# ZKTLabs/zkt-plonk

Hardware: AMD Instinct MI355X
Metric: proofs/sec (withdraw, n=2^20) (higher is better)
Workload: dtype u32 limbs (256-bit Montgomery); 1 GPU; full prove, WithdrawCircuit INPUTS=8 HEIGHT=64 Poseidon x5 (1019498 gates, 538 Poseidon gadgets), bn254, n=2^20, TABLE_SIZE=1024, 12 public inputs; parallelism=proofs sharded across 1 GPU(s), chained=True, distinct_witnesses=2, witness_on_device=True, table_cached=True, proof_bytes=802

## Files before the change

zkt-plonk_amd/csrc/kzg.hip:

```cpp
#include "ctx.hpp"
#include "hostinv.hpp"
#include "msm.hpp"
#include "poly.hpp"

#include <algorithm>
#include <cstring>
#include <functional>
#include <vector>

namespace zkt {

constexpr int KZG_OPEN_E = 4;

struct KzgState {
    hipStream_t copy = nullptr;
    hipEvent_t ev_up = nullptr, ev_main = nullptr;
    DevBuf up;
    DevBuf t, tb, w, scan, pw, part, evals;
    ~KzgState() {
        if (ev_up) (void)hipEventDestroy(ev_up);
        if (ev_main) (void)hipEventDestroy(ev_main);
        if (copy) (void)hipStreamDestroy(copy);
    }
};

static int kzg_state(zkt_ctx* c, KzgState** out) {
    if (!c->kzg) {
        auto K = std::make_shared<KzgState>();
        ZKT_HIP(c, hipStreamCreateWithFlags(&K->copy, hipStreamNonBlocking));
        ZKT_HIP(c, hipEventCreateWithFlags(&K->ev_up, hipEventDisableTiming));
        ZKT_HIP(c, hipEventCreateWithFlags(&K->ev_main, hipEventDisableTiming));
        c->kzg = K;
    }
// ... 100 lines not shown
};

template <class P>
ZKT_D Fe<P> wave_sum(Fe<P> x) {
#pragma unroll
    for (int d = 32; d >= 1; d >>= 1) {
        Fe<P> y;
#pragma unroll
        for (int w = 0; w < P::N; ++w) y.v[w] = (uint32_t)__shfl_xor((int)x.v[w], d, 64);
        x = fe_add<P>(x, y);
    }
    return x;
}

template <class P>
__global__ __launch_bounds__(256) void k_kzg_open_combine(KzgOpenArgs a, const Fe<P>* pw, const Fe<P>* blk, int fstride,
                                                         uint64_t len_max, int raw, Fe<P>* t_out, Fe<P>* partials, uint32_t nblk) {
    __shared__ Fe<P> wsum[ZKT_KZG_BATCH_MAX][4];
    const int t = threadIdx.x, lane = t & 63, wave = t >> 6;
    const uint64_t base = (uint64_t)blockIdx.x * 256 * KZG_OPEN_E;
    const Fe<P> z256 = fe_load<P>(pw + 256), zt = fe_load<P>(pw + t);
    Fe<P> acc[KZG_OPEN_E];
#pragma unroll
    for (int e = 0; e < KZG_OPEN_E; ++e) acc[e] = fe_zero<P>();
#pragma unroll 1
    for (int j = 0; j < a.nterms; ++j) {
        const uint64_t len = a.len[j];
        if (base >= len) {
            if (lane == 0) wsum[j][wave] = fe_zero<P>();
            continue;
        }
        const Fe<P>* p = (const Fe<P>*)a.poly[j];
        Fe<P> cj;
#pragma unroll
        for (int w = 0; w < P::N; ++w) cj.v[w] = a.ch[j][w];
        Fe<P> h = fe_zero<P>();
#pragma unroll
        for (int e = KZG_OPEN_E - 1; e >= 0; --e) {
            const uint64_t i = base + (uint64_t)e * 256 + t;
            const Fe<P> v = i < len ? fe_load<P>(p + i) : fe_zero<P>();
            h = fe_add<P>(fe_mul<P>(h, z256), v);
            acc[e] = fe_add<P>(acc[e], fe_mul<P>(cj, v));
        }
        h = wave_sum<P>(fe_mul<P>(h, zt));
        if (lane == 0) wsum[j][wave] = h;
    }
    const Fe<P> zb = fe_load<P>(blk + (size_t)fstride * blockIdx.x);
    Fe<P> r = fe_mul<P>(zb, zt);
#pragma unroll
    for (int e = 0; e < KZG_OPEN_E; ++e) {
        const uint64_t i = base + (uint64_t)e * 256 + t;
        if (i < len_max) fe_store<P>(t_out + i, raw ? acc[e] : fe_mul<P>(acc[e], r));
        r = fe_mul<P>(r, z256);
    }
    __syncthreads();
    if (t < a.nterms) {
        Fe<P> s = fe_add<P>(fe_add<P>(wsum[t][0], wsum[t][1]), fe_add<P>(wsum[t][2], wsum[t][3]));
        fe_store<P>(partials + (size_t)t * nblk + blockIdx.x, fe_mul<P>(s, zb));
    }
}

template <class P>
static int open_combine_t(zkt_ctx* c, const KzgOpenArgs& a, const void* pw, size_t len_max, int raw, void* t_out, void* partials,
                          uint32_t nblk) {
    const Fe<P>* tab = (const Fe<P>*)pw;
    const int fstride = KZG_OPEN_E / open_elems(len_max);
    hipLaunchKernelGGL(k_kzg_open_combine<P>, dim3(nblk), dim3(256), 0, c->stream, a, tab, tab + 2 * OPEN_PW_ROW, fstride, (uint64_t)len_max,
                       raw, (Fe<P>*)t_out, (Fe<P>*)partials, nblk);
    ZKT_HIP(c, hipGetLastError());
    return ZKT_OK;
}

template <class P>
static void inv_host(const uint32_t* z, uint32_t* zi) {
    Fe<P> x;
    memcpy(x.v, z, 32);
    x = fe_inv_host<P>(x);
    memcpy(zi, x.v, 32);
}

static int kzg_open(zkt_ctx* c, const void* const* src, bool host, const size_t* lens, int k, const uint64_t* ch, const uint64_t* z4,
                    uint64_t* out_w, int* out_inf, uint64_t* out_evals) {
    int rc = kzg_check(c, src, lens, k, out_w);
    if (rc || k == 0) return rc;
    if (!ch || !z4) return set_err(c, ZKT_ERR_INVALID_ARGUMENT, "null pointer");
    size_t L = 0, total = 0;
    for (int j = 0; j < k; ++j) {
        L = std::max(L, lens[j]);
        total += lens[j];
    }
    if (L > 0 && open_elems(L) > KZG_OPEN_E)
        return set_err(c, ZKT_ERR_INVALID_ARGUMENT, "zkt_kzg_open: polynomials longer than 2^26 coefficients");
    const int W = 2 * fq_limbs(c);
    std::vector<uint64_t> w(W, 0), ev((size_t)k * 4, 0);
    if (L == 0) {
        memcpy(out_w, w.data(), W * 8);
        if (out_inf) *out_inf = 1;
        if (out_evals) memcpy(out_evals, ev.data(), ev.size() * 8);
        return ZKT_OK;
    }
    (void)hipSetDevice(c->device);
    KzgState* K = nullptr;
    if ((rc = kzg_state(c, &K))) return rc;
    const uint32_t nblk = (uint32_t)((L + 256 * KZG_OPEN_E - 1) / (256 * KZG_OPEN_E));
    if ((rc = grow(c, K->t, L * 32)) || (rc = grow(c, K->tb, L * 32)) || (rc = grow(c, K->w, L * 32)) ||
        (rc = grow(c, K->scan, (2 * (L / 1024 + 2048)) * 32)) || (rc = grow(c, K->pw, open_witness_powers(L) * 32)) ||
        (rc = grow(c, K->part, (size_t)k * nblk * 32)) || (rc = grow(c, K->evals, (size_t)k * 32)))
        return rc;
    if (host && (rc = grow(c, K->up, total * 32))) return rc;
    KzgOpenArgs a{};
    a.nterms = k;
    size_t off = 0;
    for (int j = 0; j < k; ++j) {
        a.poly[j] = host ? (const void*)((char*)K->up.p + off) : src[j];
        a.len[j] = lens[j];
        memcpy(a.ch[j], ch + 4 * (size_t)j, 32);
        off += lens[j] * 32;
    }
    if (host) {
        if ((rc = kzg_copy_after_main(c, *K))) return rc;
        ProfScope prof(c, "kzg_open_upload", K->copy);
        for (int j = 0; j < k && !rc; ++j)
            if (lens[j]) rc = kzg_upload(c, *K, src[j], lens[j] * 32, const_cast<void*>(a.poly[j]));
        if (rc) return rc;
    }
    uint32_t z[8], zi[8] = {};
    memcpy(z, z4, 32);
    bool zero = true;
    for (int i = 0; i < 8; ++i) zero = zero && z[i] == 0;
    if (!zero) {
        if (c->curve == ZKT_CURVE_BN254) inv_host<Bn254Fr>(z, zi);
        else inv_host<Bls381Fr>(z, zi);
    }
    {
        ProfScope prof(c, "kzg_open_combine");
        if ((rc = open_pow_tables(c, z, zi, K->pw.p, L))) return rc;
        rc = c->curve == ZKT_CURVE_BN254 ? open_combine_t<Bn254Fr>(c, a, K->pw.p, L, zero, K->t.p, K->part.p, nblk)
                                         : open_combine_t<Bls381Fr>(c, a, K->pw.p, L, zero, K->t.p, K->part.p, nblk);
        if (rc) return rc;
        if (out_evals && (rc = poly_sum_rows(c, K->part.p, (int)nblk, k, K->evals.p))) return rc;
    }
    int inf = 1;
    if (L >= 2) {
        const void* scalars = (const char*)K->t.p + 32;
        if (!zero) {
            ProfScope prof(c, "kzg_open_divide");
            if ((rc = open_divide(c, K->t.p, L, K->tb.p, K->scan.p, K->w.p, K->pw.p))) return rc;
            scalars = K->w.p;
        }
        ProfScope prof(c, "kzg_open_msm");
        if ((rc = msm_g1_dev(c, scalars, L - 1, 0, 1, w.data(), &inf))) return rc;
    }
    if (out_evals) ZKT_HIP(c, hipMemcpyAsync(ev.data(), K->evals.p, (size_t)k * 32, hipMemcpyDeviceToHost, c->stream));
    ZKT_HIP(c, hipStreamSynchronize(c->stream));
    memcpy(out_w, w.data(), W * 8);
    if (out_inf) *out_inf = inf;
    if (out_evals) memcpy(out_evals, ev.data(), ev.size() * 8);
    return ZKT_OK;
}

}

// ... 24 lines not shown
```

zkt-plonk_amd/csrc/poly.hip:

```cpp
#include "poly.hpp"
#include "hostinv.hpp"

namespace zkt {

template <class P>
ZKT_D Fe<P> arg_fe(const uint32_t* w) {
    Fe<P> r;
#pragma unroll
    for (int i = 0; i < 8; ++i) r.v[i] = w[i];
    return r;
}

template <class P>
__global__ void k_mul_vec(const Fe<P>* a, const Fe<P>* b, Fe<P>* o, size_t n) {
    size_t i = (size_t)blockIdx.x * blockDim.x + threadIdx.x;
    if (i < n) fe_store<P>(o + i, fe_mul<P>(fe_load<P>(a + i), fe_load<P>(b + i)));
}

template <class P>
__global__ void k_trim_len(const Fe<P>* p, size_t lo, size_t n, uint32_t* len, int skip_if_set, Fe<P>* zero_at,
                           int zero_count) {
    if (zero_at && blockIdx.x == 0 && (int)threadIdx.x < zero_count) fe_store<P>(zero_at + threadIdx.x, fe_zero<P>());
    if (skip_if_set && *len != 0) return;
    size_t i = lo + (size_t)blockIdx.x * blockDim.x + threadIdx.x;
// ... 383 lines not shown

template <class P>
__global__ void k_quot_blind(Fe<P>* lo, Fe<P>* mid, Fe<P>* hi, const uint32_t* lens, const Fe<P>* b0b1, uint32_t n,
                             uint32_t* status) {
    if (threadIdx.x != 0 || blockIdx.x != 0) return;
    if (lens[3] > 3 * (n + 2)) { atomicOr(status, 2u); return; }
    if (lens[1] == 0 || lens[2] == 0) { atomicOr(status, 1u); return; }
    Fe<P> b0 = fe_load<P>(b0b1), b1 = fe_load<P>(b0b1 + 1);
    fe_store<P>(lo + lens[0], b0);
    fe_store<P>(mid, fe_sub<P>(fe_load<P>(mid), b0));
    fe_store<P>(mid + lens[1], b1);
    fe_store<P>(hi, fe_sub<P>(fe_load<P>(hi), b1));
}

constexpr int PW_E = 8;
constexpr int OW_THREADS = 1024;
static inline int ow_elems(size_t len) {
    int e = 2;
    while ((len + (size_t)256 * e - 1) / ((size_t)256 * e) > 65536) e <<= 1;
    return e;
}
static inline size_t ow_blocks(size_t len) {
    const size_t seg = (size_t)256 * ow_elems(len);
    return (len + seg - 1) / seg;
}
size_t open_witness_powers(size_t maxlen) { return 2 * (size_t)EV_PW + 2 * ow_blocks(maxlen) + 8; }

template <class P>
ZKT_D void pow_rounds(Fe<P>* tab, const Fe<P>& x, int cnt, int lt) {
    if (lt == 0) {
        tab[0] = fe_one<P>();
        tab[1] = x;
    }
    __syncthreads();
    for (int s = 1; s < cnt; s <<= 1) {
        for (int j = lt + 1; j <= s && s + j <= cnt; j += OW_THREADS / 2) tab[s + j] = fe_mul<P>(tab[s], tab[j]);
        __syncthreads();
    }
}
template <class P>
__global__ __launch_bounds__(OW_THREADS) void k_pow_tables(Fe<P> z, Fe<P> zinv, Fe<P>* pw, int nblk, int E) {
    __shared__ Fe<P> row[2][EV_PW], seg[2][EV_PW], top[2][EV_PW];
    const int half = threadIdx.x / (OW_THREADS / 2), lt = threadIdx.x % (OW_THREADS / 2);
    pow_rounds<P>(row[half], half ? zinv : z, 256, lt);
    Fe<P> y = row[half][256];
    for (int e = 1; e < E; e <<= 1) y = fe_sqr<P>(y);
    pow_rounds<P>(seg[half], y, 256, lt);
    const int ntop = (nblk + 255) / 256;
    pow_rounds<P>(top[half], seg[half][256], ntop, lt);
    for (int t = lt; t < EV_PW; t += OW_THREADS / 2) fe_store<P>(pw + half * EV_PW + t, row[half][t]);
    Fe<P>* blk = pw + 2 * EV_PW + (size_t)half * nblk;
    for (int b = lt; b < nblk; b += OW_THREADS / 2) fe_store<P>(blk + b, fe_mul<P>(seg[half][b & 255], top[half][b >> 8]));
}
template <class P>
__global__ __launch_bounds__(256) void k_mul_pow(const Fe<P>* in, Fe<P>* out, size_t n, size_t cap, const Fe<P>* pw, const Fe<P>* blk,
                                                 int E, int shift) {
    const size_t base = (size_t)blockIdx.x * 256 * E;
    Fe<P> r = fe_mul<P>(fe_load<P>(blk + blockIdx.x), fe_load<P>(pw + threadIdx.x + shift));
#pragma unroll 1
    for (int j = 0; j < E; ++j) {
        const size_t i = base + (size_t)j * 256 + threadIdx.x;
        if (i >= cap) break;
        fe_store<P>(out + i, i < n ? fe_mul<P>(fe_load<P>(in + i), r) : fe_zero<P>());
        if (j + 1 < E) r = fe_mul<P>(r, fe_load<P>(pw + 256));
    }
}

template <class P>
__global__ void k_gen_powers(Fe<P>* out, size_t n, Fe<P> base, Fe<P> scale) {
    size_t t = (size_t)blockIdx.x * blockDim.x + threadIdx.x;
    size_t i0 = t * PW_E;
    if (i0 >= n) return;
    Fe<P> pw = fe_mul<P>(scale, fe_pow_u64<P>(base, i0));
#pragma unroll 1
    for (int e = 0; e < PW_E && i0 + e < n; ++e) {
        fe_store<P>(out + i0 + e, pw);
        pw = fe_mul<P>(pw, base);
    }
}
// ... 389 lines not shown
    if ((rc = trim_len_t<P>(c, hi, chunk, lens + 2))) return rc;
    {
        const size_t lo = 3 * chunk, hi = 4 * n;
        hipLaunchKernelGGL(k_trim_len<P>, dim3(nblocks(hi - lo)), dim3(256), 0, c->stream, (const Fe<P>*)q, lo, hi, lens + 3, 0,
                           (Fe<P>*)nullptr, 0);
        ZKT_HIP(c, hipGetLastError());
    }
    hipLaunchKernelGGL(k_quot_blind<P>, dim3(1), dim3(64), 0, c->stream, (Fe<P>*)lo, (Fe<P>*)mid, (Fe<P>*)hi, lens, (const Fe<P>*)b0b1, (uint32_t)n, d_status);
    ZKT_HIP(c, hipGetLastError());
    return ZKT_OK;
}
int quotient_split_blind(zkt_ctx* c, const void* q, size_t n, const void* d_b0b1, void* q_lo, void* q_mid, void* q_hi, uint32_t* d_status) {
    ZKT_DISPATCH(c, quot_split_t, q, n, d_b0b1, q_lo, q_mid, q_hi, d_status);
}

int open_elems(size_t len) { return ow_elems(len); }
size_t open_blocks(size_t len) { return ow_blocks(len); }
template <class P> static int open_pow_tables_t(zkt_ctx* c, const uint32_t* z, const uint32_t* zinv, void* d_powers, size_t len) {
    hipLaunchKernelGGL(k_pow_tables<P>, dim3(1), dim3(OW_THREADS), 0, c->stream, host_fe<P>(z), host_fe<P>(zinv), (Fe<P>*)d_powers,
                       (int)ow_blocks(len), ow_elems(len));
    ZKT_HIP(c, hipGetLastError());
    return ZKT_OK;
}
int open_pow_tables(zkt_ctx* c, const uint32_t z[8], const uint32_t z_inv[8], void* d_powers, size_t len) {
    ZKT_DISPATCH(c, open_pow_tables_t, z, z_inv, d_powers, len);
}
template <class P> static int open_divide_t(zkt_ctx* c, const void* t, size_t len, void* tb, void* scan_tmp, void* out, const void* d_powers) {
    if (len == 0) return ZKT_OK;
    const Fe<P>* pw = (const Fe<P>*)d_powers;
    const int E = ow_elems(len);
    const unsigned blocks = (unsigned)ow_blocks(len);
    int rc = scan_t<P, OpAdd>(c, (const Fe<P>*)t, (Fe<P>*)tb, len, true, (Fe<P>*)scan_tmp);
    if (rc) return rc;
    hipLaunchKernelGGL(k_mul_pow<P>, dim3(blocks), dim3(256), 0, c->stream, (const Fe<P>*)tb + 1, (Fe<P>*)out, len - 1, len,
                       pw + EV_PW, pw + 2 * EV_PW + blocks, E, 1);
    ZKT_HIP(c, hipGetLastError());
    return ZKT_OK;
}
int open_divide(zkt_ctx* c, const void* t, size_t len, void* d_tmp, void* d_scan_tmp, void* out, const void* d_powers) {
    ZKT_DISPATCH(c, open_divide_t, t, len, d_tmp, d_scan_tmp, out, d_powers);
}

template <class P> static int open_witness_t(zkt_ctx* c, const void* p, size_t len, const uint32_t* z, const uint32_t* zinv, void* ta, void* tb, void* scan_tmp, void* out, void* d_powers) {
    if (len == 0) return ZKT_OK;
    Fe<P>* pw = (Fe<P>*)d_powers;
    const int E = ow_elems(len);
    const unsigned blocks = (unsigned)ow_blocks(len);
    int rc = open_pow_tables_t<P>(c, z, zinv, d_powers, len);
    if (rc) return rc;
    hipLaunchKernelGGL(k_mul_pow<P>, dim3(blocks), dim3(256), 0, c->stream, (const Fe<P>*)p, (Fe<P>*)ta, len, len,
                       (const Fe<P>*)pw, (const Fe<P>*)pw + 2 * EV_PW, E, 0);
    ZKT_HIP(c, hipGetLastError());
    return open_divide_t<P>(c, ta, len, tb, scan_tmp, out, d_powers);
}
int open_witness(zkt_ctx* c, const void* p, size_t len, const uint32_t z[8], const uint32_t z_inv[8], void* d_tmp_a, void* d_tmp_b, void* d_scan_tmp, void* out, void* d_powers) {
    ZKT_DISPATCH(c, open_witness_t, p, len, z, z_inv, d_tmp_a, d_tmp_b, d_scan_tmp, out, d_powers);
}

template <class P> static int sum_rows_t(zkt_ctx* c, const void* partials, int nblk, int rows, void* out) {
    hipLaunchKernelGGL(k_eval_final<P>, dim3(rows), dim3(256), 0, c->stream, (const Fe<P>*)partials, nblk, (Fe<P>*)out);
    ZKT_HIP(c, hipGetLastError());
    return ZKT_OK;
}
int poly_sum_rows(zkt_ctx* c, const void* d_partials, int nblk, int rows, void* d_out) {
    ZKT_DISPATCH(c, sum_rows_t, d_partials, nblk, rows, d_out);
}

template <class P> static int gen_powers_t(zkt_ctx* c, void* out, size_t n, const uint32_t* base, const uint32_t* scale) {
    if (!n) return ZKT_OK;
    hipLaunchKernelGGL(k_gen_powers<P>, dim3(nblocks((n + PW_E - 1) / PW_E)), dim3(256), 0, c->stream, (Fe<P>*)out, n, host_fe<P>(base), host_fe<P>(scale));
    ZKT_HIP(c, hipGetLastError());
// ... 32 lines not shown
```

zkt-plonk_amd/csrc/poly.hpp:

```cpp
#pragma once
#include "ctx.hpp"

namespace zkt {

constexpr int LC_MAX_TERMS = 16;
struct LinCombArgs {
    const void* poly[LC_MAX_TERMS];
    uint64_t len[LC_MAX_TERMS];
    uint32_t scalar[LC_MAX_TERMS][8];
    int nterms;
};

constexpr int EVAL_MAX = 16;
struct EvalArgs {
    const void* poly[EVAL_MAX];
    uint64_t len[EVAL_MAX];
    uint32_t point[EVAL_MAX][8];
    int count;
};

struct QuotientArgs {
    const void *a, *b, *c, *pi, *z1, *z2, *t, *h1, *h2;
    const void *q_m, *q_l, *q_r, *q_o, *q_c, *q_lookup, *q_table, *sigma1, *sigma2, *sigma3, *x, *l1;
    void* out;
// ... 25 lines not shown
int poly_add_blinders(zkt_ctx* c, void* p, const uint32_t* d_len, const void* d_blinders, int k, size_t cap);
int poly_lincomb(zkt_ctx* c, const LinCombArgs& a, void* out, size_t n);
int lagrange_scalars(zkt_ctx* c, const void* ev, size_t n, const uint32_t* d_len, const void* d_blinders, int k, const void* d_roots,
                     void* out);
int poly_eval_many(zkt_ctx* c, const EvalArgs& a, void* d_partials, void* d_results, void* d_powers);
int z1_terms(zkt_ctx* c, const ZTermsArgs& a);
int z2_terms(zkt_ctx* c, const ZTermsArgs& a);
int scan_mul(zkt_ctx* c, const void* in, void* out, size_t n, bool reverse, void* d_tmp );
int scan_add(zkt_ctx* c, const void* in, void* out, size_t n, bool reverse, void* d_tmp);
int z_combine(zkt_ctx* c, const void* pn, const void* sd, const uint32_t inv_total[8], void* out, size_t n);
int quotient_pointwise(zkt_ctx* c, const QuotientArgs& a);
int to_hat_form(zkt_ctx* c, void* v, size_t n, int k32);
int quotient_interleave(zkt_ctx* c, const void* in, void* out, size_t n4, uint32_t G, uint32_t chunks = 1);
int quotient_split_blind(zkt_ctx* c, const void* q, size_t n, const void* d_b0b1, void* q_lo, void* q_mid, void* q_hi,
                         uint32_t* d_status);
int open_witness(zkt_ctx* c, const void* p, size_t len, const uint32_t z[8], const uint32_t z_inv[8], void* d_tmp_a, void* d_tmp_b,
                 void* d_scan_tmp, void* out, void* d_powers );
size_t open_witness_powers(size_t maxlen);
constexpr int OPEN_PW_ROW = 257;
int open_elems(size_t len);
size_t open_blocks(size_t len);
int open_pow_tables(zkt_ctx* c, const uint32_t z[8], const uint32_t z_inv[8], void* d_powers, size_t len);
int open_divide(zkt_ctx* c, const void* t, size_t len, void* d_tmp, void* d_scan_tmp, void* out, const void* d_powers);
int poly_sum_rows(zkt_ctx* c, const void* d_partials, int nblk, int rows, void* d_out);
int gen_powers(zkt_ctx* c, void* out, size_t n, const uint32_t base[8], const uint32_t scale[8]);
int lookup_count(zkt_ctx* c, const void* f, size_t n, const void* d_sorted_keys, const uint32_t* d_perm, uint32_t nkeys,
                 uint32_t* d_counts, uint32_t* d_status);
int lookup_starts(zkt_ctx* c, const uint32_t* d_base_counts, uint32_t* d_hits, uint32_t nkeys, size_t n, uint32_t* d_even,
                  uint32_t* d_odd, uint32_t* d_status);
int lookup_expand(zkt_ctx* c, const void* d_keys_insertion, const uint32_t* d_starts, uint32_t nkeys, void* out, size_t n);

}
```

zkt-plonk_amd/csrc/prover.hip:

```cpp
#include "ctx.hpp"
#include "hostinv.hpp"
#include <chrono>
#include <cstdio>
#include <cstdlib>
#include "ec.hpp"
#include "keyfile.hpp"
#include "msm.hpp"
#include "poly.hpp"
#include "transcript.hpp"

#include <algorithm>
#include <functional>
#include <cstring>
#include <memory>
#include <optional>
#include <vector>

namespace zkt {

enum { PK_QM = 0, PK_QL, PK_QR, PK_QO, PK_QC, PK_S1, PK_S2, PK_S3, PK_QLOOKUP, PK_QTABLE, PK_COUNT };
enum { CS_QM = 0, CS_QL, CS_QR, CS_QO, CS_QC, CS_QLOOKUP, CS_QTABLE, CS_S1, CS_S2, CS_S3, CS_X, CS_L1, CS_COUNT };
enum { W_A = 0, W_B, W_C, W_PI, W_Z1, W_Z2, W_T, W_H1, W_H2, W_COUNT };

struct CircuitState {
// ... 26 lines not shown
    uint32_t lk_nkeys = 0;
    std::vector<uint32_t> lk_host_keys, lk_host_sorted, lk_host_counts, lk_host_order;
    bool has_next = false, prefetch_same_table = false;
    int prefetch_stage = 0;
    uint64_t prefetch_epoch = 0;
    zkt_prove_inputs next_in{}, prefetch_in{};
    void* poly_alt[3] = {};
    uint32_t* status_alt = nullptr;
    void* lk_keys = nullptr;
    size_t lk_cap = 0;
    void* pinned = nullptr;
    hipStream_t comm_stream = nullptr;
    hipEvent_t ev_piece[ZKT_QUOTIENT_CHUNKS] = {}, ev_gathered = nullptr;
    hipStream_t aux_stream = nullptr;
    hipEvent_t ev_aux_go = nullptr, ev_aux_done = nullptr;
    void* aux_scan_tmp = nullptr;
    void* aux_pw = nullptr;
    hipStream_t copy_stream = nullptr;
    hipEvent_t ev_copy[4] = {};
    void* pinned_pi = nullptr;
    uint32_t* pi_tab = nullptr;
    void* eval_pw = nullptr;
    std::vector<uint64_t> cached_table;
    bool t_cached = false, t_coset_valid = false;
    uint64_t t_srs_generation = 0;
    uint64_t t_commit_xy[12] = {};
    bool keys_borrowed = false;
    bool wire_route[3] = {};
    bool wire_dense_only = false;
};

template <class P>
// ... 785 lines not shown
        if ((rc = poly_lincomb(c, lr, work, cap))) return rc;
        if (fe_is_zero<R>(xi) || fe_is_zero<R>(shifted)) return set_err(c, ZKT_ERR_ZERO_DENOMINATOR, "evaluation challenge is zero");
        Affine<Q> aw, saw;
        {
            LinCombArgs lo{};
            F pw = one;
            term(lo, work, cap, pw);
            const void* ps[8] = {S.poly[0], S.poly[1], S.poly[2], S.pk[PK_S1], S.pk[PK_S2], S.pk[PK_QLOOKUP], S.poly[3], S.poly[5]};
            const size_t pl[8] = {cap, cap, cap, S.pk_len[PK_S1], S.pk_len[PK_S2], S.pk_len[PK_QLOOKUP], cap, cap};
            for (int k = 0; k < 8; ++k) {
                pw = fe_mul<R>(pw, eta);
                term(lo, ps[k], pl[k], pw);
            }
            void* comb = S.sc[0];
            if ((rc = poly_lincomb(c, lo, comb, cap))) return rc;
            F zi = fe_inv_host<R>(xi);
            if ((rc = open_witness(c, comb, cap, xi.v, zi.v, S.sc[1], S.sc[2], S.scan_tmp, S.sc[3], S.eval_pw))) return rc;
        }
        const bool aux = S.aux_stream != nullptr && !c->aux_off;
        void* comb2 = aux ? S.wcos[W_Z1] : S.sc[0];
        void* ta2 = aux ? (void*)((char*)S.wcos[W_Z1] + cap * 32) : S.sc[1];
        void* tb2 = aux ? (void*)((char*)S.wcos[W_Z1] + 2 * cap * 32) : S.sc[2];
        void* out2 = aux ? S.wcos[W_Z2] : S.sc[3];
        auto second_opening = [&]() -> int {
            LinCombArgs lo{};
            F pw = one;
            const void* ps[4] = {S.poly[6], S.poly[7], S.poly[3], S.poly[4]};
            for (int k = 0; k < 4; ++k) {
                term(lo, ps[k], cap, pw);
                pw = fe_mul<R>(pw, eta);
            }
            int r2;
            if ((r2 = poly_lincomb(c, lo, comb2, cap))) return r2;
            F zi = fe_inv_host<R>(shifted);
            return open_witness(c, comb2, cap, shifted.v, zi.v, ta2, tb2, aux ? S.aux_scan_tmp : S.scan_tmp, out2,
                                aux ? S.aux_pw : S.eval_pw);
        };
        if (aux) {
            ZKT_HIP(c, hipEventRecord(S.ev_aux_go, c->stream));
            ZKT_HIP(c, hipStreamWaitEvent(S.aux_stream, S.ev_aux_go, 0));
            hipStream_t main_stream = c->stream;
            c->stream = S.aux_stream;
            const int r2 = second_opening();
            c->stream = main_stream;
            if (r2) return r2;
            ZKT_HIP(c, hipEventRecord(S.ev_aux_done, S.aux_stream));
        }
        const bool both = aux && queueing();
        if (!both && (rc = commit_begin(S.sc[3], cap - 1, 6))) return rc;
        {
            if (aux) ZKT_HIP(c, hipStreamWaitEvent(c->stream, S.ev_aux_done, 0));
// ... 58 lines not shown
    if (!S.keys_borrowed) {
        for (void* p : S.pk) fr(p);
        for (void* p : S.coset) fr(p);
        for (void* p : S.sigma_ev) fr(p);
        fr(S.q_lookup_ev); fr(S.roots);
    }
    for (void* p : S.ev) fr(p);
    for (void* p : S.sc) fr(p);
    fr(S.scan_tmp);
    for (void* p : S.poly) fr(p);
    for (void* p : S.wcos) fr(p);
    for (void* p : S.wnext) fr(p);
    fr(S.fold); fr(S.qgather);
    for (void* p : S.poly_alt) fr(p);
    fr(S.status_alt);
    fr(S.aux_scan_tmp); fr(S.aux_pw);
    for (void* q : S.lag_scalars_q) fr(q);
    wire_bases_drop(c);
    if (S.aux_stream) {
        (void)hipStreamSynchronize(S.aux_stream);
        (void)hipStreamDestroy(S.aux_stream);
    }
    if (S.ev_aux_go) (void)hipEventDestroy(S.ev_aux_go);
    if (S.ev_aux_done) (void)hipEventDestroy(S.ev_aux_done);
    fr(S.qev); fr(S.small); fr(S.lag_scalars); fr(S.status); fr(S.lk_u32); fr(S.lk_keys); fr(S.pi_tab); fr(S.eval_pw);
    if (S.pinned) (void)hipHostFree(S.pinned);
    if (S.pinned_pi) (void)hipHostFree(S.pinned_pi);
    if (S.copy_stream) {
        (void)hipStreamSynchronize(S.copy_stream);
        (void)hipStreamDestroy(S.copy_stream);
    }
// ... 31 lines not shown
    if ((rc = dev_alloc(c, (void**)&S.status_alt, 64 * 4))) return rc;
    for (auto& p : S.poly_alt) if ((rc = alloc(&p, n + 8))) return rc;
    S.lk_cap = n + 2;
    if ((rc = dev_alloc(c, (void**)&S.lk_u32, 5 * S.lk_cap * 4 + 16))) return rc;
    if ((rc = alloc(&S.lk_keys, 2 * S.lk_cap))) return rc;
    ZKT_HIP(c, hipHostMalloc(&S.pinned, 64 * 32));
    ZKT_HIP(c, hipStreamCreateWithFlags(&S.copy_stream, hipStreamNonBlocking));
    if (S.G > 1) {
        ZKT_HIP(c, hipStreamCreateWithFlags(&S.comm_stream, hipStreamNonBlocking));
        for (auto& e : S.ev_piece) ZKT_HIP(c, hipEventCreateWithFlags(&e, hipEventDisableTiming));
        ZKT_HIP(c, hipEventCreateWithFlags(&S.ev_gathered, hipEventDisableTiming));
    }
    for (auto& e : S.ev_copy) ZKT_HIP(c, hipEventCreateWithFlags(&e, hipEventDisableTiming));
    ZKT_HIP(c, hipHostMalloc(&S.pinned_pi, QUOTIENT_PI_DIRECT_MAX * 40));
    if ((rc = dev_alloc(c, (void**)&S.pi_tab, QUOTIENT_PI_DIRECT_MAX * 40))) return rc;
    if ((rc = alloc(&S.eval_pw, std::max((size_t)EVAL_MAX * (257 + eval_blocks), open_witness_powers(n + 8))))) return rc;
    if (S.G == 1) {
        if ((rc = alloc(&S.aux_scan_tmp, 2 * ((n + 8) / 1024 + 4096)))) return rc;
        if ((rc = alloc(&S.aux_pw, open_witness_powers(n + 8)))) return rc;
        ZKT_HIP(c, hipStreamCreateWithFlags(&S.aux_stream, hipStreamNonBlocking));
        ZKT_HIP(c, hipEventCreateWithFlags(&S.ev_aux_go, hipEventDisableTiming));
        ZKT_HIP(c, hipEventCreateWithFlags(&S.ev_aux_done, hipEventDisableTiming));
    }
    return ZKT_OK;
}

int circuit_fork(zkt_ctx* child, const zkt_ctx* parent) {
    circuit_release(child);
    if (!parent->circuit) return ZKT_OK;
    const CircuitState& P0 = *parent->circuit;
    auto st = std::make_shared<CircuitState>();
    CircuitState& S = *st;
    S.log_n = P0.log_n; S.n = P0.n; S.G = P0.G; S.cls = P0.cls; S.log_m = P0.log_m; S.m = P0.m;
    for (int k = 0; k < PK_COUNT; ++k) { S.pk[k] = P0.pk[k]; S.pk_len[k] = P0.pk_len[k]; }
// ... 643 lines not shown
    void* d_partials = (char*)S.small + 64 * 32;
    void* d_results = (char*)S.small + 32 * 32;
    int rc = poly_eval_many(c, ea, d_partials, d_results, S.eval_pw);
    if (rc) return rc;
    if ((rc = poly_lincomb(c, lc, S.sc[0], out_len))) return rc;
    ZKT_HIP(c, hipMemcpyAsync(out_evals, d_results, (size_t)k * 32, hipMemcpyDeviceToHost, c->stream));
    ZKT_HIP(c, hipMemcpyAsync(out_lincomb, S.sc[0], out_len * 32, hipMemcpyDeviceToHost, c->stream));
    ZKT_HIP(c, hipStreamSynchronize(c->stream));
    return ZKT_OK;
}

int zkt_debug_open_witness(zkt_ctx* c, const uint64_t* coeffs, size_t len, const uint64_t* z4, uint64_t* out) {
    if (!c || !coeffs || !z4 || !out) return set_err(c, ZKT_ERR_INVALID_ARGUMENT, "null pointer");
    if (!c->circuit) return set_err(c, ZKT_ERR_NOT_LOADED, "no circuit loaded (zkt_circuit_load)");
    CircuitState& S = *c->circuit;
    if (len < 2 || len > S.n + 8) return set_err(c, ZKT_ERR_INVALID_ARGUMENT, "2 .. n + 8 coefficients");
    (void)hipSetDevice(c->device);
    c->circuit->prefetch_stage = 0;
    uint32_t z[8], zi[8];
    memcpy(z, z4, 32);
    bool zero = true;
    for (int i = 0; i < 8; ++i) zero = zero && z[i] == 0;
    if (zero) return set_err(c, ZKT_ERR_ZERO_DENOMINATOR, "evaluation point is zero");
    if (c->curve == ZKT_CURVE_BN254) {
        Fe<Bn254Fr> x;
        memcpy(x.v, z, 32);
        x = fe_inv_host<Bn254Fr>(x);
        memcpy(zi, x.v, 32);
    } else {
        Fe<Bls381Fr> x;
        memcpy(x.v, z, 32);
        x = fe_inv_host<Bls381Fr>(x);
        memcpy(zi, x.v, 32);
    }
    ZKT_HIP(c, hipMemcpyAsync(S.sc[0], coeffs, len * 32, hipMemcpyHostToDevice, c->stream));
    int rc = open_witness(c, S.sc[0], len, z, zi, S.sc[1], S.sc[2], S.scan_tmp, S.sc[3], S.eval_pw);
    if (rc) return rc;
    ZKT_HIP(c, hipMemcpyAsync(out, S.sc[3], (len - 1) * 32, hipMemcpyDeviceToHost, c->stream));
    ZKT_HIP(c, hipStreamSynchronize(c->stream));
    return ZKT_OK;
}

extern "C++" template <class C>
static int debug_commit_wires_t(zkt_ctx* c, const zkt_prove_inputs& in, int route, uint64_t* out_xy, int* out_inf, int* out_route) {
    using Q = typename C::Fq;
    CircuitState& S = *c->circuit;
    MerlinHostTranscript tr("zkt_debug_commit_wires_dev");
    Prover<C> p(c, S, tr);
    S.wire_dense_only = route == 0;
    int rc = p.enqueue_round_1(in);
    S.wire_dense_only = false;
    Affine<Q> cm[3];
    static const int slots[3] = {0, 1, 2};
    int took[3] = {0, 0, 0};
// ... 72 lines not shown
```

Before: 56.77 proofs/s.

## Replace inverse-scaled prefix scan in KZG opening with Horner-based synthetic division

The KZG witness computation used to scale the coefficients by powers of z, run a generic prefix scan, then rescale by powers of z^-1, which needed a host inversion and several full passes. It now divides by (X - z) directly, in three steps: a per-block Horner suffix scan with precomputed power ladders, a single-block carry scan across blocks, and a quotient kernel. This drops the pre-multiply and post-multiply passes, the host inversion and two scratch buffers. In exchange the carry step runs serially in one block, and the batched open kernel loses its raw/scaled mode.

After: 56.34 proofs/s. Within noise of the previous version (-0.8%).

```diff
diff --git a/zkt-plonk_amd/csrc/kzg.hip b/zkt-plonk_amd/csrc/kzg.hip
--- a/zkt-plonk_amd/csrc/kzg.hip
+++ b/zkt-plonk_amd/csrc/kzg.hip
@@ -1,5 +1,4 @@
 #include "ctx.hpp"
-#include "hostinv.hpp"
 #include "msm.hpp"
 #include "poly.hpp"
 
@@ -16,7 +15,7 @@
     hipStream_t copy = nullptr;
     hipEvent_t ev_up = nullptr, ev_main = nullptr;
     DevBuf up;
-    DevBuf t, tb, w, scan, pw, part, evals;
+    DevBuf t, w, scratch, pw, part, evals;
     ~KzgState() {
         if (ev_up) (void)hipEventDestroy(ev_up);
         if (ev_main) (void)hipEventDestroy(ev_main);
@@ -147,8 +146,8 @@
 }
 
 template <class P>
-__global__ __launch_bounds__(256) void k_kzg_open_combine(KzgOpenArgs a, const Fe<P>* pw, const Fe<P>* blk, int fstride,
-                                                         uint64_t len_max, int raw, Fe<P>* t_out, Fe<P>* partials, uint32_t nblk) {
+__global__ __launch_bounds__(256) void k_kzg_open_combine(KzgOpenArgs a, const Fe<P>* pw, const Fe<P>* blk, uint64_t len_max,
+                                                         Fe<P>* t_out, Fe<P>* partials, uint32_t nblk) {
     __shared__ Fe<P> wsum[ZKT_KZG_BATCH_MAX][4];
     const int t = threadIdx.x, lane = t & 63, wave = t >> 6;
     const uint64_t base = (uint64_t)blockIdx.x * 256 * KZG_OPEN_E;
@@ -178,13 +177,11 @@
         h = wave_sum<P>(fe_mul<P>(h, zt));
         if (lane == 0) wsum[j][wave] = h;
     }
-    const Fe<P> zb = fe_load<P>(blk + (size_t)fstride * blockIdx.x);
-    Fe<P> r = fe_mul<P>(zb, zt);
+    const Fe<P> zb = fe_load<P>(blk + blockIdx.x);
 #pragma unroll
     for (int e = 0; e < KZG_OPEN_E; ++e) {
         const uint64_t i = base + (uint64_t)e * 256 + t;
-        if (i < len_max) fe_store<P>(t_out + i, raw ? acc[e] : fe_mul<P>(acc[e], r));
-        r = fe_mul<P>(r, z256);
+        if (i < len_max) fe_store<P>(t_out + i, acc[e]);
     }
     __syncthreads();
     if (t < a.nterms) {
@@ -194,22 +191,13 @@
 }
 
 template <class P>
-static int open_combine_t(zkt_ctx* c, const KzgOpenArgs& a, const void* pw, size_t len_max, int raw, void* t_out, void* partials,
+static int open_combine_t(zkt_ctx* c, const KzgOpenArgs& a, const void* pw, size_t len_max, void* t_out, void* partials,
                           uint32_t nblk) {
     const Fe<P>* tab = (const Fe<P>*)pw;
-    const int fstride = KZG_OPEN_E / open_elems(len_max);
-    hipLaunchKernelGGL(k_kzg_open_combine<P>, dim3(nblk), dim3(256), 0, c->stream, a, tab, tab + 2 * OPEN_PW_ROW, fstride, (uint64_t)len_max,
-                       raw, (Fe<P>*)t_out, (Fe<P>*)partials, nblk);
+    hipLaunchKernelGGL(k_kzg_open_combine<P>, dim3(nblk), dim3(256), 0, c->stream, a, tab, tab + OPEN_PW_ROW, (uint64_t)len_max,
+                       (Fe<P>*)t_out, (Fe<P>*)partials, nblk);
     ZKT_HIP(c, hipGetLastError());
     return ZKT_OK;
-}
-
-template <class P>
-static void inv_host(const uint32_t* z, uint32_t* zi) {
-    Fe<P> x;
-    memcpy(x.v, z, 32);
-    x = fe_inv_host<P>(x);
-    memcpy(zi, x.v, 32);
 }
 
 static int kzg_open(zkt_ctx* c, const void* const* src, bool host, const size_t* lens, int k, const uint64_t* ch, const uint64_t* z4,
@@ -222,7 +210,7 @@
         L = std::max(L, lens[j]);
         total += lens[j];
     }
-    if (L > 0 && open_elems(L) > KZG_OPEN_E)
+    if (L > ((size_t)1 << 26))
         return set_err(c, ZKT_ERR_INVALID_ARGUMENT, "zkt_kzg_open: polynomials longer than 2^26 coefficients");
     const int W = 2 * fq_limbs(c);
     std::vector<uint64_t> w(W, 0), ev((size_t)k * 4, 0);
@@ -236,8 +224,8 @@
     KzgState* K = nullptr;
     if ((rc = kzg_state(c, &K))) return rc;
     const uint32_t nblk = (uint32_t)((L + 256 * KZG_OPEN_E - 1) / (256 * KZG_OPEN_E));
-    if ((rc = grow(c, K->t, L * 32)) || (rc = grow(c, K->tb, L * 32)) || (rc = grow(c, K->w, L * 32)) ||
-        (rc = grow(c, K->scan, (2 * (L / 1024 + 2048)) * 32)) || (rc = grow(c, K->pw, open_witness_powers(L) * 32)) ||
+    if ((rc = grow(c, K->t, L * 32)) || (rc = grow(c, K->w, L * 32)) ||
+        (rc = grow(c, K->scratch, open_witness_scratch(L) * 32)) || (rc = grow(c, K->pw, ((size_t)OPEN_PW_ROW + nblk) * 32)) ||
         (rc = grow(c, K->part, (size_t)k * nblk * 32)) || (rc = grow(c, K->evals, (size_t)k * 32)))
         return rc;
     if (host && (rc = grow(c, K->up, total * 32))) return rc;
@@ -257,19 +245,15 @@
             if (lens[j]) rc = kzg_upload(c, *K, src[j], lens[j] * 32, const_cast<void*>(a.poly[j]));
         if (rc) return rc;
     }
-    uint32_t z[8], zi[8] = {};
+    uint32_t z[8];
     memcpy(z, z4, 32);
     bool zero = true;
     for (int i = 0; i < 8; ++i) zero = zero && z[i] == 0;
-    if (!zero) {
-        if (c->curve == ZKT_CURVE_BN254) inv_host<Bn254Fr>(z, zi);
-        else inv_host<Bls381Fr>(z, zi);
-    }
     {
         ProfScope prof(c, "kzg_open_combine");
-        if ((rc = open_pow_tables(c, z, zi, K->pw.p, L))) return rc;
-        rc = c->curve == ZKT_CURVE_BN254 ? open_combine_t<Bn254Fr>(c, a, K->pw.p, L, zero, K->t.p, K->part.p, nblk)
-                                         : open_combine_t<Bls381Fr>(c, a, K->pw.p, L, zero, K->t.p, K->part.p, nblk);
+        if ((rc = open_pow_tables(c, z, K->pw.p, (int)nblk, KZG_OPEN_E))) return rc;
+        rc = c->curve == ZKT_CURVE_BN254 ? open_combine_t<Bn254Fr>(c, a, K->pw.p, L, K->t.p, K->part.p, nblk)
+                                         : open_combine_t<Bls381Fr>(c, a, K->pw.p, L, K->t.p, K->part.p, nblk);
         if (rc) return rc;
         if (out_evals && (rc = poly_sum_rows(c, K->part.p, (int)nblk, k, K->evals.p))) return rc;
     }
@@ -278,7 +262,7 @@
         const void* scalars = (const char*)K->t.p + 32;
         if (!zero) {
             ProfScope prof(c, "kzg_open_divide");
-            if ((rc = open_divide(c, K->t.p, L, K->tb.p, K->scan.p, K->w.p, K->pw.p))) return rc;
+            if ((rc = open_witness(c, K->t.p, L, z, K->scratch.p, K->w.p))) return rc;
             scalars = K->w.p;
         }
         ProfScope prof(c, "kzg_open_msm");
diff --git a/zkt-plonk_amd/csrc/poly.hip b/zkt-plonk_amd/csrc/poly.hip
--- a/zkt-plonk_amd/csrc/poly.hip
+++ b/zkt-plonk_amd/csrc/poly.hip
@@ -421,55 +421,130 @@
 }
 
 constexpr int PW_E = 8;
-constexpr int OW_THREADS = 1024;
-static inline int ow_elems(size_t len) {
-    int e = 2;
-    while ((len + (size_t)256 * e - 1) / ((size_t)256 * e) > 65536) e <<= 1;
-    return e;
-}
-static inline size_t ow_blocks(size_t len) {
-    const size_t seg = (size_t)256 * ow_elems(len);
-    return (len + seg - 1) / seg;
-}
-size_t open_witness_powers(size_t maxlen) { return 2 * (size_t)EV_PW + 2 * ow_blocks(maxlen) + 8; }
-
-template <class P>
-ZKT_D void pow_rounds(Fe<P>* tab, const Fe<P>& x, int cnt, int lt) {
-    if (lt == 0) {
+#ifndef ZKT_OPEN_E
+#define ZKT_OPEN_E 8
+#endif
+constexpr int OW_E = ZKT_OPEN_E;
+constexpr int OW_T = 256;
+constexpr int OW_LOG_T = 8;
+constexpr int OW_B = OW_E * OW_T;
+constexpr int OW_CT = 512;
+constexpr int OW_LOG_CT = 9;
+static_assert((1 << OW_LOG_T) == OW_T && (1 << OW_LOG_CT) == OW_CT && (OW_E & (OW_E - 1)) == 0, "powers of two");
+static inline size_t ow_blocks(size_t len) { return (len + OW_B - 1) / OW_B; }
+size_t open_witness_scratch(size_t maxlen) { return ow_blocks(maxlen) * OW_T + ow_blocks(maxlen) + OW_T + 1; }
+
+template <class P>
+struct OpenPowers {
+    Fe<P> z;
+    Fe<P> run[OW_LOG_T];
+    Fe<P> blk[OW_LOG_CT];
+};
+
+template <class P>
+ZKT_D void pow_rounds(Fe<P>* tab, const Fe<P>& x, int cnt) {
+    if (threadIdx.x == 0) {
         tab[0] = fe_one<P>();
         tab[1] = x;
     }
     __syncthreads();
     for (int s = 1; s < cnt; s <<= 1) {
-        for (int j = lt + 1; j <= s && s + j <= cnt; j += OW_THREADS / 2) tab[s + j] = fe_mul<P>(tab[s], tab[j]);
-        __syncthreads();
-    }
-}
-template <class P>
-__global__ __launch_bounds__(OW_THREADS) void k_pow_tables(Fe<P> z, Fe<P> zinv, Fe<P>* pw, int nblk, int E) {
-    __shared__ Fe<P> row[2][EV_PW], seg[2][EV_PW], top[2][EV_PW];
-    const int half = threadIdx.x / (OW_THREADS / 2), lt = threadIdx.x % (OW_THREADS / 2);
-    pow_rounds<P>(row[half], half ? zinv : z, 256, lt);
-    Fe<P> y = row[half][256];
+        for (int j = threadIdx.x + 1; j <= s && s + j <= cnt; j += blockDim.x) tab[s + j] = fe_mul<P>(tab[s], tab[j]);
+        __syncthreads();
+    }
+}
+constexpr int PT_THREADS = 512;
+template <class P>
+__global__ __launch_bounds__(PT_THREADS) void k_pow_tables(Fe<P> z, Fe<P>* pw, int nblk, int E) {
+    __shared__ Fe<P> row[EV_PW], seg[EV_PW], top[EV_PW];
+    pow_rounds<P>(row, z, 256);
+    Fe<P> y = row[256];
     for (int e = 1; e < E; e <<= 1) y = fe_sqr<P>(y);
-    pow_rounds<P>(seg[half], y, 256, lt);
+    pow_rounds<P>(seg, y, 256);
     const int ntop = (nblk + 255) / 256;
-    pow_rounds<P>(top[half], seg[half][256], ntop, lt);
-    for (int t = lt; t < EV_PW; t += OW_THREADS / 2) fe_store<P>(pw + half * EV_PW + t, row[half][t]);
-    Fe<P>* blk = pw + 2 * EV_PW + (size_t)half * nblk;
-    for (int b = lt; b < nblk; b += OW_THREADS / 2) fe_store<P>(blk + b, fe_mul<P>(seg[half][b & 255], top[half][b >> 8]));
-}
-template <class P>
-__global__ __launch_bounds__(256) void k_mul_pow(const Fe<P>* in, Fe<P>* out, size_t n, size_t cap, const Fe<P>* pw, const Fe<P>* blk,
-                                                 int E, int shift) {
-    const size_t base = (size_t)blockIdx.x * 256 * E;
-    Fe<P> r = fe_mul<P>(fe_load<P>(blk + blockIdx.x), fe_load<P>(pw + threadIdx.x + shift));
+    pow_rounds<P>(top, seg[256], ntop);
+    for (int t = threadIdx.x; t < EV_PW; t += PT_THREADS) fe_store<P>(pw + t, row[t]);
+    Fe<P>* blk = pw + EV_PW;
+    for (int b = threadIdx.x; b < nblk; b += PT_THREADS) fe_store<P>(blk + b, fe_mul<P>(seg[b & 255], top[b >> 8]));
+}
+
+template <class P>
+__global__ __launch_bounds__(OW_T) void k_open_partials(const Fe<P>* p, size_t len, OpenPowers<P> pw, Fe<P>* suf) {
+    __shared__ Fe<P> u[OW_T];
+    const int t = threadIdx.x;
+    const size_t s = ((size_t)blockIdx.x * OW_T + t) * OW_E;
+    Fe<P> c[OW_E];
+#pragma unroll
+    for (int e = 0; e < OW_E; ++e) c[e] = s + e < len ? fe_load<P>(p + s + e) : fe_zero<P>();
+    Fe<P> h = c[OW_E - 1];
+#pragma unroll
+    for (int e = OW_E - 2; e >= 0; --e) h = fe_add<P>(fe_mul<P>(h, pw.z), c[e]);
+    u[t] = h;
+    __syncthreads();
 #pragma unroll 1
-    for (int j = 0; j < E; ++j) {
-        const size_t i = base + (size_t)j * 256 + threadIdx.x;
-        if (i >= cap) break;
-        fe_store<P>(out + i, i < n ? fe_mul<P>(fe_load<P>(in + i), r) : fe_zero<P>());
-        if (j + 1 < E) r = fe_mul<P>(r, fe_load<P>(pw + 256));
+    for (int k = 0; k < OW_LOG_T; ++k) {
+        const int d = 1 << k;
+        const bool live = t + d < OW_T;
+        Fe<P> add = fe_zero<P>();
+        if (live) add = fe_mul<P>(u[t + d], pw.run[k]);
+        __syncthreads();
+        if (live) {
+            h = fe_add<P>(h, add);
+            u[t] = h;
+        }
+        __syncthreads();
+    }
+    fe_store<P>(suf + (size_t)blockIdx.x * OW_T + t, h);
+}
+
+template <class P>
+__global__ __launch_bounds__(OW_CT) void k_open_carries(const Fe<P>* suf, int nblk, OpenPowers<P> pw, Fe<P>* carry, Fe<P>* tab) {
+    __shared__ Fe<P> row[OW_T + 1];
+    __shared__ Fe<P> v[OW_CT];
+    const int t = threadIdx.x;
+    pow_rounds<P>(row, pw.run[0], OW_T);
+    for (int k = t; k <= OW_T; k += OW_CT) fe_store<P>(tab + k, row[k]);
+    Fe<P> top = fe_zero<P>();
+    for (int lo = (nblk - 1) / OW_CT * OW_CT; lo >= 0; lo -= OW_CT) {
+        const int b = lo + t;
+        Fe<P> x = b + 1 < nblk ? fe_load<P>(suf + (size_t)(b + 1) * OW_T) : fe_zero<P>();
+        if (t == OW_CT - 1) x = fe_add<P>(x, fe_mul<P>(top, pw.blk[0]));
+        v[t] = x;
+        __syncthreads();
+#pragma unroll 1
+        for (int k = 0; k < OW_LOG_CT; ++k) {
+            const int d = 1 << k;
+            const bool live = t + d < OW_CT;
+            Fe<P> add = fe_zero<P>();
+            if (live) add = fe_mul<P>(v[t + d], pw.blk[k]);
+            __syncthreads();
+            if (live) {
+                x = fe_add<P>(x, add);
+                v[t] = x;
+            }
+            __syncthreads();
+        }
+        if (b < nblk) fe_store<P>(carry + b, x);
+        top = v[0];
+        __syncthreads();
+    }
+}
+
+template <class P>
+__global__ __launch_bounds__(OW_T) void k_open_quotient(const Fe<P>* p, size_t len, Fe<P> z, const Fe<P>* suf, const Fe<P>* carry,
+                                                        const Fe<P>* tab, Fe<P>* out) {
+    const int t = threadIdx.x;
+    const size_t s = ((size_t)blockIdx.x * OW_T + t) * OW_E;
+    if (s >= len) return;
+    Fe<P> c[OW_E];
+#pragma unroll
+    for (int e = 1; e < OW_E; ++e) c[e] = s + e < len ? fe_load<P>(p + s + e) : fe_zero<P>();
+    Fe<P> q = fe_mul<P>(fe_load<P>(carry + blockIdx.x), fe_load<P>(tab + (OW_T - 1 - t)));
+    if (t + 1 < OW_T) q = fe_add<P>(q, fe_load<P>(suf + (size_t)blockIdx.x * OW_T + t + 1));
+#pragma unroll
+    for (int e = OW_E - 1; e >= 0; --e) {
+        if (s + e < len) fe_store<P>(out + s + e, q);
+        if (e) q = fe_add<P>(fe_mul<P>(q, z), c[e]);
     }
 }
 
@@ -889,47 +964,40 @@
     ZKT_DISPATCH(c, quot_split_t, q, n, d_b0b1, q_lo, q_mid, q_hi, d_status);
 }
 
-int open_elems(size_t len) { return ow_elems(len); }
-size_t open_blocks(size_t len) { return ow_blocks(len); }
-template <class P> static int open_pow_tables_t(zkt_ctx* c, const uint32_t* z, const uint32_t* zinv, void* d_powers, size_t len) {
-    hipLaunchKernelGGL(k_pow_tables<P>, dim3(1), dim3(OW_THREADS), 0, c->stream, host_fe<P>(z), host_fe<P>(zinv), (Fe<P>*)d_powers,
-                       (int)ow_blocks(len), ow_elems(len));
-    ZKT_HIP(c, hipGetLastError());
-    return ZKT_OK;
-}
-int open_pow_tables(zkt_ctx* c, const uint32_t z[8], const uint32_t z_inv[8], void* d_powers, size_t len) {
-    ZKT_DISPATCH(c, open_pow_tables_t, z, z_inv, d_powers, len);
-}
-template <class P> static int open_divide_t(zkt_ctx* c, const void* t, size_t len, void* tb, void* scan_tmp, void* out, const void* d_powers) {
+template <class P> static int open_pow_tables_t(zkt_ctx* c, const uint32_t* z, void* d_powers, int nblk, int E) {
+    if (nblk > 256 * 256) return set_err(c, ZKT_ERR_INVALID_ARGUMENT, "open_pow_tables: more than 65536 block powers");
+    hipLaunchKernelGGL(k_pow_tables<P>, dim3(1), dim3(PT_THREADS), 0, c->stream, host_fe<P>(z), (Fe<P>*)d_powers, nblk, E);
+    ZKT_HIP(c, hipGetLastError());
+    return ZKT_OK;
+}
+int open_pow_tables(zkt_ctx* c, const uint32_t z[8], void* d_powers, int nblk, int E) {
+    ZKT_DISPATCH(c, open_pow_tables_t, z, d_powers, nblk, E);
+}
+
+template <class P> static int open_witness_t(zkt_ctx* c, const void* p, size_t len, const uint32_t* z, void* d_scratch, void* out) {
     if (len == 0) return ZKT_OK;
-    const Fe<P>* pw = (const Fe<P>*)d_powers;
-    const int E = ow_elems(len);
-    const unsigned blocks = (unsigned)ow_blocks(len);
-    int rc = scan_t<P, OpAdd>(c, (const Fe<P>*)t, (Fe<P>*)tb, len, true, (Fe<P>*)scan_tmp);
-    if (rc) return rc;
-    hipLaunchKernelGGL(k_mul_pow<P>, dim3(blocks), dim3(256), 0, c->stream, (const Fe<P>*)tb + 1, (Fe<P>*)out, len - 1, len,
-                       pw + EV_PW, pw + 2 * EV_PW + blocks, E, 1);
-    ZKT_HIP(c, hipGetLastError());
-    return ZKT_OK;
-}
-int open_divide(zkt_ctx* c, const void* t, size_t len, void* d_tmp, void* d_scan_tmp, void* out, const void* d_powers) {
-    ZKT_DISPATCH(c, open_divide_t, t, len, d_tmp, d_scan_tmp, out, d_powers);
-}
-
-template <class P> static int open_witness_t(zkt_ctx* c, const void* p, size_t len, const uint32_t* z, const uint32_t* zinv, void* ta, void* tb, void* scan_tmp, void* out, void* d_powers) {
-    if (len == 0) return ZKT_OK;
-    Fe<P>* pw = (Fe<P>*)d_powers;
-    const int E = ow_elems(len);
-    const unsigned blocks = (unsigned)ow_blocks(len);
-    int rc = open_pow_tables_t<P>(c, z, zinv, d_powers, len);
-    if (rc) return rc;
-    hipLaunchKernelGGL(k_mul_pow<P>, dim3(blocks), dim3(256), 0, c->stream, (const Fe<P>*)p, (Fe<P>*)ta, len, len,
-                       (const Fe<P>*)pw, (const Fe<P>*)pw + 2 * EV_PW, E, 0);
-    ZKT_HIP(c, hipGetLastError());
-    return open_divide_t<P>(c, ta, len, tb, scan_tmp, out, d_powers);
-}
-int open_witness(zkt_ctx* c, const void* p, size_t len, const uint32_t z[8], const uint32_t z_inv[8], void* d_tmp_a, void* d_tmp_b, void* d_scan_tmp, void* out, void* d_powers) {
-    ZKT_DISPATCH(c, open_witness_t, p, len, z, z_inv, d_tmp_a, d_tmp_b, d_scan_tmp, out, d_powers);
+    const size_t nblk = ow_blocks(len);
+    if (nblk > 0x7fffffffu / OW_T) return set_err(c, ZKT_ERR_INVALID_ARGUMENT, "open_witness: polynomial too long");
+    OpenPowers<P> pw;
+    pw.z = host_fe<P>(z);
+    Fe<P> y = pw.z;
+    for (int e = 1; e < OW_E; e <<= 1) y = fe_sqr<P>(y);
+    for (int s = 0; s < OW_LOG_T; ++s, y = fe_sqr<P>(y)) pw.run[s] = y;
+    for (int s = 0; s < OW_LOG_CT; ++s, y = fe_sqr<P>(y)) pw.blk[s] = y;
+    Fe<P>* suf = (Fe<P>*)d_scratch;
+    Fe<P>* carry = suf + nblk * OW_T;
+    Fe<P>* tab = carry + nblk;
+    hipLaunchKernelGGL(k_open_partials<P>, dim3((unsigned)nblk), dim3(OW_T), 0, c->stream, (const Fe<P>*)p, len, pw, suf);
+    ZKT_HIP(c, hipGetLastError());
+    hipLaunchKernelGGL(k_open_carries<P>, dim3(1), dim3(OW_CT), 0, c->stream, (const Fe<P>*)suf, (int)nblk, pw, carry, tab);
+    ZKT_HIP(c, hipGetLastError());
+    hipLaunchKernelGGL(k_open_quotient<P>, dim3((unsigned)nblk), dim3(OW_T), 0, c->stream, (const Fe<P>*)p, len, pw.z,
+                       (const Fe<P>*)suf, (const Fe<P>*)carry, (const Fe<P>*)tab, (Fe<P>*)out);
+    ZKT_HIP(c, hipGetLastError());
+    return ZKT_OK;
+}
+int open_witness(zkt_ctx* c, const void* p, size_t len, const uint32_t z[8], void* d_scratch, void* out) {
+    ZKT_DISPATCH(c, open_witness_t, p, len, z, d_scratch, out);
 }
 
 template <class P> static int sum_rows_t(zkt_ctx* c, const void* partials, int nblk, int rows, void* out) {
diff --git a/zkt-plonk_amd/csrc/poly.hpp b/zkt-plonk_amd/csrc/poly.hpp
--- a/zkt-plonk_amd/csrc/poly.hpp
+++ b/zkt-plonk_amd/csrc/poly.hpp
@@ -63,14 +63,10 @@
 int quotient_interleave(zkt_ctx* c, const void* in, void* out, size_t n4, uint32_t G, uint32_t chunks = 1);
 int quotient_split_blind(zkt_ctx* c, const void* q, size_t n, const void* d_b0b1, void* q_lo, void* q_mid, void* q_hi,
                          uint32_t* d_status);
-int open_witness(zkt_ctx* c, const void* p, size_t len, const uint32_t z[8], const uint32_t z_inv[8], void* d_tmp_a, void* d_tmp_b,
-                 void* d_scan_tmp, void* out, void* d_powers );
-size_t open_witness_powers(size_t maxlen);
+int open_witness(zkt_ctx* c, const void* p, size_t len, const uint32_t z[8], void* d_scratch, void* out);
+size_t open_witness_scratch(size_t maxlen);
 constexpr int OPEN_PW_ROW = 257;
-int open_elems(size_t len);
-size_t open_blocks(size_t len);
-int open_pow_tables(zkt_ctx* c, const uint32_t z[8], const uint32_t z_inv[8], void* d_powers, size_t len);
-int open_divide(zkt_ctx* c, const void* t, size_t len, void* d_tmp, void* d_scan_tmp, void* out, const void* d_powers);
+int open_pow_tables(zkt_ctx* c, const uint32_t z[8], void* d_powers, int nblk, int E);
 int poly_sum_rows(zkt_ctx* c, const void* d_partials, int nblk, int rows, void* d_out);
 int gen_powers(zkt_ctx* c, void* out, size_t n, const uint32_t base[8], const uint32_t scale[8]);
 int lookup_count(zkt_ctx* c, const void* f, size_t n, const void* d_sorted_keys, const uint32_t* d_perm, uint32_t nkeys,
diff --git a/zkt-plonk_amd/csrc/prover.hip b/zkt-plonk_amd/csrc/prover.hip
--- a/zkt-plonk_amd/csrc/prover.hip
+++ b/zkt-plonk_amd/csrc/prover.hip
@@ -64,8 +64,7 @@
     hipEvent_t ev_piece[ZKT_QUOTIENT_CHUNKS] = {}, ev_gathered = nullptr;
     hipStream_t aux_stream = nullptr;
     hipEvent_t ev_aux_go = nullptr, ev_aux_done = nullptr;
-    void* aux_scan_tmp = nullptr;
-    void* aux_pw = nullptr;
+    void* open_tmp[2] = {nullptr, nullptr};
     hipStream_t copy_stream = nullptr;
     hipEvent_t ev_copy[4] = {};
     void* pinned_pi = nullptr;
@@ -881,13 +880,10 @@
             }
             void* comb = S.sc[0];
             if ((rc = poly_lincomb(c, lo, comb, cap))) return rc;
-            F zi = fe_inv_host<R>(xi);
-            if ((rc = open_witness(c, comb, cap, xi.v, zi.v, S.sc[1], S.sc[2], S.scan_tmp, S.sc[3], S.eval_pw))) return rc;
+            if ((rc = open_witness(c, comb, cap, xi.v, S.open_tmp[0], S.sc[3]))) return rc;
         }
         const bool aux = S.aux_stream != nullptr && !c->aux_off;
         void* comb2 = aux ? S.wcos[W_Z1] : S.sc[0];
-        void* ta2 = aux ? (void*)((char*)S.wcos[W_Z1] + cap * 32) : S.sc[1];
-        void* tb2 = aux ? (void*)((char*)S.wcos[W_Z1] + 2 * cap * 32) : S.sc[2];
         void* out2 = aux ? S.wcos[W_Z2] : S.sc[3];
         auto second_opening = [&]() -> int {
             LinCombArgs lo{};
@@ -899,9 +895,7 @@
             }
             int r2;
             if ((r2 = poly_lincomb(c, lo, comb2, cap))) return r2;
-            F zi = fe_inv_host<R>(shifted);
-            return open_witness(c, comb2, cap, shifted.v, zi.v, ta2, tb2, aux ? S.aux_scan_tmp : S.scan_tmp, out2,
-                                aux ? S.aux_pw : S.eval_pw);
+            return open_witness(c, comb2, cap, shifted.v, S.open_tmp[1], out2);
         };
         if (aux) {
             ZKT_HIP(c, hipEventRecord(S.ev_aux_go, c->stream));
@@ -990,7 +984,7 @@
     fr(S.fold); fr(S.qgather);
     for (void* p : S.poly_alt) fr(p);
     fr(S.status_alt);
-    fr(S.aux_scan_tmp); fr(S.aux_pw);
+    for (void* p : S.open_tmp) fr(p);
     for (void* q : S.lag_scalars_q) fr(q);
     wire_bases_drop(c);
     if (S.aux_stream) {
@@ -1052,10 +1046,9 @@
     for (auto& e : S.ev_copy) ZKT_HIP(c, hipEventCreateWithFlags(&e, hipEventDisableTiming));
     ZKT_HIP(c, hipHostMalloc(&S.pinned_pi, QUOTIENT_PI_DIRECT_MAX * 40));
     if ((rc = dev_alloc(c, (void**)&S.pi_tab, QUOTIENT_PI_DIRECT_MAX * 40))) return rc;
-    if ((rc = alloc(&S.eval_pw, std::max((size_t)EVAL_MAX * (257 + eval_blocks), open_witness_powers(n + 8))))) return rc;
+    if ((rc = alloc(&S.eval_pw, (size_t)EVAL_MAX * (257 + eval_blocks)))) return rc;
+    for (auto& p : S.open_tmp) if ((rc = alloc(&p, open_witness_scratch(n + 8)))) return rc;
     if (S.G == 1) {
-        if ((rc = alloc(&S.aux_scan_tmp, 2 * ((n + 8) / 1024 + 4096)))) return rc;
-        if ((rc = alloc(&S.aux_pw, open_witness_powers(n + 8)))) return rc;
         ZKT_HIP(c, hipStreamCreateWithFlags(&S.aux_stream, hipStreamNonBlocking));
         ZKT_HIP(c, hipEventCreateWithFlags(&S.ev_aux_go, hipEventDisableTiming));
         ZKT_HIP(c, hipEventCreateWithFlags(&S.ev_aux_done, hipEventDisableTiming));
@@ -1729,30 +1722,30 @@
     if (!c || !coeffs || !z4 || !out) return set_err(c, ZKT_ERR_INVALID_ARGUMENT, "null pointer");
     if (!c->circuit) return set_err(c, ZKT_ERR_NOT_LOADED, "no circuit loaded (zkt_circuit_load)");
     CircuitState& S = *c->circuit;
-    if (len < 2 || len > S.n + 8) return set_err(c, ZKT_ERR_INVALID_ARGUMENT, "2 .. n + 8 coefficients");
+    if (len < 1) return set_err(c, ZKT_ERR_INVALID_ARGUMENT, "at least one coefficient");
     (void)hipSetDevice(c->device);
     c->circuit->prefetch_stage = 0;
-    uint32_t z[8], zi[8];
+    uint32_t z[8];
     memcpy(z, z4, 32);
-    bool zero = true;
-    for (int i = 0; i < 8; ++i) zero = zero && z[i] == 0;
-    if (zero) return set_err(c, ZKT_ERR_ZERO_DENOMINATOR, "evaluation point is zero");
-    if (c->curve == ZKT_CURVE_BN254) {
-        Fe<Bn254Fr> x;
-        memcpy(x.v, z, 32);
-        x = fe_inv_host<Bn254Fr>(x);
-        memcpy(zi, x.v, 32);
-    } else {
-        Fe<Bls381Fr> x;
-        memcpy(x.v, z, 32);
-        x = fe_inv_host<Bls381Fr>(x);
-        memcpy(zi, x.v, 32);
-    }
-    ZKT_HIP(c, hipMemcpyAsync(S.sc[0], coeffs, len * 32, hipMemcpyHostToDevice, c->stream));
-    int rc = open_witness(c, S.sc[0], len, z, zi, S.sc[1], S.sc[2], S.scan_tmp, S.sc[3], S.eval_pw);
+    void *in = S.sc[0], *tmp = S.open_tmp[0], *res = S.sc[3];
+    void* own[3] = {nullptr, nullptr, nullptr};
+    int rc = ZKT_OK;
+    if (len > S.n + 8) {
+        if ((rc = dev_alloc(c, &own[0], len * 32)) || (rc = dev_alloc(c, &own[1], open_witness_scratch(len) * 32)) ||
+            (rc = dev_alloc(c, &own[2], len * 32))) {
+            for (void* p : own) dev_free(c, p);
+            return rc;
+        }
+        in = own[0]; tmp = own[1]; res = own[2];
+    }
+    hipError_t e = hipMemcpyAsync(in, coeffs, len * 32, hipMemcpyHostToDevice, c->stream);
+    if (e == hipSuccess) rc = open_witness(c, in, len, z, tmp, res);
+    if (e == hipSuccess && !rc && len > 1) e = hipMemcpyAsync(out, res, (len - 1) * 32, hipMemcpyDeviceToHost, c->stream);
+    const hipError_t e2 = hipStreamSynchronize(c->stream);
+    for (void* p : own) dev_free(c, p);
     if (rc) return rc;
-    ZKT_HIP(c, hipMemcpyAsync(out, S.sc[3], (len - 1) * 32, hipMemcpyDeviceToHost, c->stream));
-    ZKT_HIP(c, hipStreamSynchronize(c->stream));
+    ZKT_HIP(c, e);
+    ZKT_HIP(c, e2);
     return ZKT_OK;
 }
 
```
